# castorini/howl

Hardware: AMD Instinct MI355X
Metric: utterances/sec/node (res8 end-to-end training step, 1s@16kHz, 40-mel) (higher is better)
Workload: dtype f32; 1 GPU; res8 training step (frontend+fwd+xent+bwd+AdamW), 512 x 1 s utterances per GPU, 12 labels -- BASELINE configs[2] per-GPU share: res8 GSC-12, 512 x 1 s per GPU (4096 over 8); global_batch=512, samples_per_utterance=16000, labels=12, parallelism=single, frontend=eval

## Files before the change

howl_amd/csrc/res8.hip:

```cpp
#include "howl_common.hip.h"
#include "../../include/howl_hip.h"

namespace {

struct HowlPtrs6 {
    float* p[6];
};
constexpr int MAX_WINDOWS = 64;
struct HowlWinRows {
    int lo[MAX_WINDOWS], hi[MAX_WINDOWS];
};
struct HowlBnBuffers {
    float* running_mean;
    float* running_var;
    long long* num_batches;
};
struct BnFold {
    const float* part;
    int nparts;
    double count;
    float* stats_out;
    HowlBnBuffers bn;
};

// ... 519 lines not shown
        SlotVal v[3];
        SlotVal ge[3];
        int bsl = b, bnsl = bn, pv = P;
        bool zb = false, zn = false;
        if constexpr (HALO == 2) {
            const StripPos pb = strip_pos(gx.sg, b, P / PW), pn = strip_pos(gx.sg, more ? bn : b, P / PW);
            bsl = pb.bu, bnsl = pn.bu, pv = pb.hv * PW;
            zb = pb.hv < P / PW, zn = pn.hv < P / PW;
        }
        f32x4 acc[NTV];
        KCursor<NTV> k;
        if constexpr (NTW > 0) k_begin<NTW, TS>(k, acc, c.ltile, c.wnt, c.CS, P, c.t0, lane);
        if constexpr (NTW > 0) k_prime<NTW>(k);
        constexpr bool STAGE = true;
        const int a0 = 2, a1 = 2, a2 = KG_A - 4, b0 = 2, b1 = 2, b2 = KG_B - 4;
#define HOWL_WINO_CHUNK() ((void)0)
#define HOWL_WINO_BAR() ((void)0)
        if constexpr (STAGE) {
            slot_load<MODE, HALO>(v[0], cfg, ubase + r1, tid, pk1[0], bsl);
            slot_load<MODE, HALO>(v[1], cfg, ubase + r1, tid + CONV_THREADS, pk1[1], bsl);
            if constexpr (HALO == 1) halo_load<MODE>(v[2], cfg, (size_t)(b ^ 1) * NMAP * P, hs[1], gcol, b);
            if constexpr (HALO == 2) grid_load<MODE>(ge, cfg, gx, 1, b, P / PW, P);
        }
        HOWL_STAIR(3);
        HOWL_WINO_CHUNK();
        if constexpr (NTW > 0) k_run<NTW>(k, acc, c.CS, a0);
        HOWL_WINO_BAR();
        if constexpr (STAGE) {
            slot_write<MODE>(v[0], cfg, ubase + r1, tid, pk1[0], c.tile, c.lm, HALO == 2 && zb && ((gx.pad[1] >> 0) & 1));
            slot_write<MODE>(v[1], cfg, ubase + r1, tid + CONV_THREADS, pk1[1], c.tile, c.lm, HALO == 2 && zb && ((gx.pad[1] >> 1) & 1));
            if constexpr (HALO == 1) halo_write<MODE>(v[2], cfg, hs[1], lcol, c.tile, c.lm);
            if constexpr (HALO == 2) grid_write<MODE>(ge, cfg, gx, 1, b, P / PW, c.tile, c.lm);
            slot_load<MODE, HALO>(v[0], cfg, ubase + r1, tid + 2 * CONV_THREADS, pk1[2], bsl);
            slot_load<MODE, HALO>(v[1], cfg, ubase + r1, tid + 3 * CONV_THREADS, pk1[3], bsl);
        }
        HOWL_STAIR(2);
        HOWL_WINO_CHUNK();
        if constexpr (NTW > 0) k_run<NTW>(k, acc, c.CS, a1);
        HOWL_WINO_BAR();
        if constexpr (STAGE) {
            slot_write<MODE>(v[0], cfg, ubase + r1, tid + 2 * CONV_THREADS, pk1[2], c.tile, c.lm, HALO == 2 && zb && ((gx.pad[1] >> 2) & 1));
            slot_write<MODE>(v[1], cfg, ubase + r1, tid + 3 * CONV_THREADS, pk1[3], c.tile, c.lm, HALO == 2 && zb && ((gx.pad[1] >> 3) & 1));
        }
        HOWL_STAIR(1);
        HOWL_WINO_CHUNK();
        if constexpr (NTW > 0) k_run<NTW>(k, acc, c.CS, a2);
        HOWL_WINO_BAR();
        HOWL_STAIR(0);
        __syncthreads();
        if constexpr (NTW > 0) k_prime<NTW>(k);
        if (STAGE && more) {
            slot_load<MODE, HALO>(v[0], cfg, nbase, tid, pk0[0], bnsl);
            slot_load<MODE, HALO>(v[1], cfg, nbase, tid + CONV_THREADS, pk0[1], bnsl);
            slot_load<MODE, HALO>(v[2], cfg, nbase, tid + 2 * CONV_THREADS, pk0[2], bnsl);
            if constexpr (HALO == 2) grid_load<MODE>(ge, cfg, gx, 0, bn, P / PW, P);
        }
        HOWL_STAIR(3);
        HOWL_WINO_CHUNK();
        if constexpr (NTW > 0) k_run<NTW>(k, acc, c.CS, b0);
        HOWL_WINO_BAR();
        if (STAGE && more) {
            slot_write<MODE>(v[0], cfg, nbase, tid, pk0[0], c.tile, c.lm, HALO == 2 && zn && ((gx.pad[0] >> 0) & 1));
            slot_write<MODE>(v[1], cfg, nbase, tid + CONV_THREADS, pk0[1], c.tile, c.lm, HALO == 2 && zn && ((gx.pad[0] >> 1) & 1));
            slot_write<MODE>(v[2], cfg, nbase, tid + 2 * CONV_THREADS, pk0[2], c.tile, c.lm, HALO == 2 && zn && ((gx.pad[0] >> 2) & 1));
            if constexpr (HALO == 2) grid_write<MODE>(ge, cfg, gx, 0, bn, P / PW, c.tile, c.lm);
            slot_load<MODE, HALO>(v[0], cfg, nbase, tid + 3 * CONV_THREADS, pk0[3], bnsl);
            slot_load<MODE, HALO>(v[1], cfg, nbase, tid + 4 * CONV_THREADS, pk0[4], bnsl);
            if constexpr (HALO == 1) halo_load<MODE>(v[2], cfg, (size_t)(bn ^ 1) * NMAP * P, hs[0], gcol, bn);
        }
        HOWL_STAIR(2);
        HOWL_WINO_CHUNK();
        if constexpr (NTW > 0) k_run<NTW>(k, acc, c.CS, b1);
        HOWL_WINO_BAR();
        if (STAGE && more) {
            slot_write<MODE>(v[0], cfg, nbase, tid + 3 * CONV_THREADS, pk0[3], c.tile, c.lm, HALO == 2 && zn && ((gx.pad[0] >> 3) & 1));
            slot_write<MODE>(v[1], cfg, nbase, tid + 4 * CONV_THREADS, pk0[4], c.tile, c.lm, HALO == 2 && zn && ((gx.pad[0] >> 4) & 1));
            if constexpr (HALO == 1) halo_write<MODE>(v[2], cfg, hs[0], lcol, c.tile, c.lm);
        }
        float2 ev[NTV][2];
        if constexpr (NTW > 0) {
            if (eop != nullptr) {
                const EpiAddr<NTW, TS> ea(epi, c.t0, lane);
                const char* ebase = reinterpret_cast<const char*>(eop + ubase);
#pragma unroll
                for (int i = 0; i < NTW; ++i)
#pragma unroll
                    for (int hh = 0; hh < 2; ++hh) ev[i][hh] = *reinterpret_cast<const float2*>(ebase + ea.off(i, hh));
            }
// ... 1 lines not shown
            k_run<NTW>(k, acc, c.CS, b2);
            k_tail<NTW>(k, acc, dl);
            HOWL_STAIR(0);
        }
        if constexpr (NTW > 0) conv_epilogue<MODE, NTW, TS, HALO>(acc, ev, epi, ubase, c.t0, lane, st0, st1, b, pv);
        __syncthreads();
    }
}

struct BwdFold {
    const float* stats;
    const float* m12;
    const float* part;
    int nparts;
    double count;
};
__device__ __forceinline__ void bwd_consts_to_lds(float* lm, int ch, float mean, float rstd, float m1, float m2) {
    lm[ch] = rstd;
    lm[CP + ch] = -rstd * rstd * m2;
    lm[2 * CP + ch] = rstd * (mean * rstd * m2 - m1);
}
__device__ __forceinline__ void bwd_fold_to_lds(float* lm, const BwdFold& f, int tid, int nthreads) {
    const int lane = tid & 63, wave = tid >> 6;
    if (f.part == nullptr) {
        if (tid < CP) bwd_consts_to_lds(lm, tid, f.stats[tid], f.stats[CP + tid], f.m12[tid], f.m12[CP + tid]);
    } else {
        const int c8 = lane >> 3;
        for (int ch0 = 4 * wave; ch0 < CP; ch0 += 4 * (nthreads >> 6)) {
            const int ch = ch0 + (c8 & 3);
            const float mean = f.stats[ch], rstd = f.stats[CP + ch];
            const double acc = fold_part_column(f.part, part_stride(f.nparts), f.nparts, (c8 < 4 ? 0 : CP) + ch, lane);
            const double second = __shfl_xor(acc, 32);
            if (c8 < 4 && (lane & 7) == 0)
                bwd_consts_to_lds(lm, ch, mean, rstd, (float)(acc / f.count), (float)(second / f.count));
        }
    }
}

struct WFold {
// ... 98 lines not shown
                const float fr = (ch < NMAP) ? (float)(1.0 / sqrt(var + (double)BN_EPS)) : 0.0f;
                lm[ch] = -fm * fr;
                lm[CP + ch] = fr;
                if (bid == 0 && slice == 0) {
                    fold.stats_out[ch] = fm;
                    fold.stats_out[CP + ch] = fr;
                    if (ch < NMAP && fold.bn.running_mean != nullptr) {
                        const double unbiased = fold.count > 1.0 ? var * fold.count / (fold.count - 1.0) : var;
                        fold.bn.running_mean[ch] = (1.0f - BN_MOMENTUM) * fold.bn.running_mean[ch] + BN_MOMENTUM * (float)mean;
                        fold.bn.running_var[ch] = (1.0f - BN_MOMENTUM) * fold.bn.running_var[ch] + BN_MOMENTUM * (float)unbiased;
                    }
                    if (ch == 0 && fold.bn.num_batches != nullptr) fold.bn.num_batches[0] += 1;
                }
            }
        }
        if (MODE == 1 && cfg.fused) bwd_fold_to_lds(lm, bfold, tid, CONV_THREADS);
        zero_lds(tile, TF, tid, CONV_THREADS);
#pragma unroll
        for (int j = 0; j < 7; ++j) {
            const int i = tid + j * CONV_THREADS;
            if (i < 3 * KSTEPS * 16) reinterpret_cast<float4*>(wl)[i] = wv[j];
        }
    }
    if (MODE == 0 && !folding && tid < CP) {
        lm[tid] = cfg.affine ? -in_stats[tid] * in_stats[CP + tid] : 0.0f;
        lm[CP + tid] = cfg.affine ? in_stats[CP + tid] : 1.0f;
    }
    const int cout = 16 * nt + (lane & 15);
    const bool cvalid = cout < NMAP;
    float xshift = 0.0f, xrstd = 1.0f;
    if (MODE == 1 && xs != nullptr && xs_stats != nullptr && cvalid) {
// ... 541 lines not shown
    WSlot first[WNT];
    if (b < B) {
#pragma unroll
        for (int j = 0; j < WNT; ++j) {
            wz_load<HALO>(first[j].z, st.z, (size_t)b * NMAP * P, zt[j], ct[j], HALO == 2 ? strip_pos(sg, b, H).bu : b);
            wx_load(first[j].x, st.x, (size_t)b * NMAP * P, xt[j]);
        }
    }
    float firsth = 0.0f, firstr = 0.0f;
    if constexpr (HALO != 0) {
        if (b < B) firsth = whalo_load(st.x, (size_t)(b ^ 1) * NMAP * P, wh[0], (b & 1) ? PW - 1 : 0);
    }
    if constexpr (HALO == 2) {
        if (b < B) firstr = wrow_load(st.x, gx, b, H, P, false);
    }
    zero_lds(lds, tile_floats_z(H) + tile_floats_x(H), tid, CONV_THREADS);
    if (st.z.fused) {
        bwd_fold_to_lds(lm, bfold, tid, CONV_THREADS);
    }
    if (tid < CP) {
        lm[4 * CP + tid] = st.xaffine ? -in_stats[tid] * in_stats[CP + tid] : 0.0f;
        lm[5 * CP + tid] = st.xaffine ? in_stats[CP + tid] : 1.0f;
    }
    __syncthreads();
    if (b < B) {
#pragma unroll
        for (int j = 0; j < WNT; ++j) {
            const bool padded = HALO == 2 && strip_pos(sg, b, H).hv < H;
            wz_write(first[j].z, st.z, zt[j], ct[j], tz, lm, padded && ((gx.pzt >> j) & 1));
            wx_write(first[j].x, st.xaffine, xt[j], ct[j], tx, lm, padded && ((gx.pxt >> j) & 1));
// ... 53 lines not shown
    if (r < SD)
        conv3x3_body<1, SD, HALO>(zc, nullptr, wp, nullptr, dx, xs, xs_stats, spart, nullptr, B, H, j, nblk, r, BnFold{}, bfold, wf, sg);
    else
        wgrad_body<SW, HALO>(WStage{zc, s_prev, false}, in_stats, bfold, wpart, B, H, j, nblk, r - SD, sg);
}

struct RowsAdamW {
    float* p;
    const float* g0;
    float* m;
    float* v;
    HowlAdamWCoef c;
    long rest_lo, rest_hi;
    int on;
};
__device__ __forceinline__ void reduce_rows_body(const float* __restrict__ part, int nparts, int ncols, int mode,
                                                 float* __restrict__ out, const RowsAdamW& opt) {
    __shared__ float red[16][64];
    const int lane = threadIdx.x & 63, rg = threadIdx.x >> 6, nrg = blockDim.x >> 6;
    const int col = blockIdx.x * 64 + lane;
    float s = 0.0f;
    if (col < ncols) {
        const float* src = part + col;
        for (int g = rg; g < nparts; g += 8 * nrg) {
            float v[8];
#pragma unroll
            for (int u = 0; u < 8; ++u) {
                const int r = g + u * nrg;
                v[u] = src[(size_t)(r < nparts ? r : nparts - 1) * ncols];
            }
// ... 8 lines not shown
        for (int r = 1; r < nrg; ++r) tot += red[r][lane];
        long d = -1;
        if (mode == 0) {
            d = col;
        } else {
            const int co = col / WNCOL, idx = col - co * WNCOL;
            if (co < NMAP && idx < WTAPS) d = (co * NMAP + idx % NMAP) * 9 + idx / NMAP;
        }
        if (d >= 0) {
            out[d] = tot;
            if (opt.on) howl_adamw_element(opt.p, opt.m, opt.v, (size_t)((out - opt.g0) + d), tot, opt.c);
        }
    }
}

__global__ __launch_bounds__(1024) void reduce_rows_all_kernel(const float* __restrict__ part, size_t layer_stride, int nparts,
                                                              HowlPtrs6 out, const float* __restrict__ c0part, int c0parts,
                                                              float* __restrict__ c0out, int y0, int yskip, int nrows, RowsAdamW opt) {
    if ((int)blockIdx.y >= nrows) {
        for (long i = opt.rest_lo + (long)blockIdx.x * blockDim.x + threadIdx.x; i < opt.rest_hi; i += (long)gridDim.x * blockDim.x)
            howl_adamw_element(opt.p, opt.m, opt.v, (size_t)i, opt.g0[i], opt.c);
        return;
    }
    const int y = y0 + (int)blockIdx.y * (1 + yskip);
    if (y < 6) {
        reduce_rows_body(part + y * layer_stride, nparts, CP * WNCOL, 1, out.p[y], opt);
    } else if (blockIdx.x * 64 < NMAP * 9) {
        reduce_rows_body(c0part, c0parts, NMAP * 9, 0, c0out, opt);
    }
}

__global__ void bn_eval_stats_kernel(HowlPtrs6 rmean, HowlPtrs6 rvar, float* __restrict__ stats) {
    const int layer = blockIdx.x, c = threadIdx.x;
// ... 288 lines not shown
                    }
            }
        }
    }
#pragma unroll
    for (int j = 0; j < C0G_CPW; ++j)
#pragma unroll
        for (int t = 0; t < 9; ++t) {
            const float v = wave_sum_rows(acc[j][t]);
            if (lane == 0) part[(size_t)blockIdx.x * NMAP * 9 + (C0G_CPW * wave + j) * 9 + t] = v;
        }
}

constexpr int HEAD_XC = 64;
constexpr int HEAD_THREADS = 768, HEAD_PARTS = 16;
__global__ __launch_bounds__(HEAD_THREADS) void head_fwd_kernel(const float* __restrict__ s6, const float* __restrict__ stats,
                                                       const float* __restrict__ wout, const float* __restrict__ bout,
                                                       float* __restrict__ pooled, float* __restrict__ logits, int B,
                                                       int P, int C, const long long* __restrict__ labels,
                                                       float* __restrict__ nll, float* __restrict__ dlogits,
                                                       float* __restrict__ dpool, float inv_batch,
                                                       const float* __restrict__ pool, int npg, int npg_used, BnFold fold,
                                                       int ns ) {
    __shared__ float lp[CP];
    __shared__ float ll[HEAD_XC], dl[HEAD_XC], lse_s;
    __shared__ float lst[2 * CP];
    __shared__ float lw[HEAD_XC * NMAP];
    __shared__ float lparts[HEAD_PARTS][CP];
    const int tid = threadIdx.x, lane = tid & 63, wave = tid >> 6;
    const bool w_in_lds = C <= HEAD_XC;
    if (w_in_lds)
        for (int i = tid; i < C * NMAP; i += HEAD_THREADS) lw[i] = wout[i];
    if (fold.part != nullptr) {
        const int c8 = lane >> 3;
        for (int w0 = wave; w0 < CP / 4; w0 += HEAD_THREADS / 64) {
            const int c = 4 * w0 + (c8 & 3);
            const double sm = fold_part_column(fold.part, part_stride(fold.nparts), fold.nparts, (c8 < 4 ? 0 : CP) + c, lane);
            const double q = __shfl_xor(sm, 32);
            if (c8 < 4 && (lane & 7) == 0) {
                const double mean = sm / fold.count;
                double var = q / fold.count - mean * mean;
                var = var < 0.0 ? 0.0 : var;
                const float fm = (c < NMAP) ? (float)mean : 0.0f;
                const float fr = (c < NMAP) ? (float)(1.0 / sqrt(var + (double)BN_EPS)) : 0.0f;
                lst[c] = fm;
                lst[CP + c] = fr;
                if (blockIdx.x == 0) {
                    fold.stats_out[c] = fm;
                    fold.stats_out[CP + c] = fr;
                    if (c < NMAP && fold.bn.running_mean != nullptr) {
                        const double unbiased = fold.count > 1.0 ? var * fold.count / (fold.count - 1.0) : var;
                        fold.bn.running_mean[c] = (1.0f - BN_MOMENTUM) * fold.bn.running_mean[c] + BN_MOMENTUM * (float)mean;
                        fold.bn.running_var[c] = (1.0f - BN_MOMENTUM) * fold.bn.running_var[c] + BN_MOMENTUM * (float)unbiased;
                    }
                    if (c == 0 && fold.bn.num_batches != nullptr) fold.bn.num_batches[0] += 1;
                }
            }
        }
    } else if (tid < 2 * CP) {
        lst[tid] = stats[tid];
    }
    __syncthreads();
    for (int b = blockIdx.x; b < B; b += gridDim.x) {
        __syncthreads();
        if (pool != nullptr) {
            const int nparts = ns * npg_used;
            const int pc = tid % CP, pk = tid / CP;
            float acc = 0.0f;
            for (int k0 = 0; k0 < nparts; k0 += HEAD_PARTS) {
                const int k = k0 + pk;
                if (k < nparts) {
                    const int sgi = k / npg_used, g = k - sgi * npg_used;
                    lparts[pk][pc] = pool[(((size_t)b * ns + sgi) * npg + g) * CP + pc];
                }
                __syncthreads();
                if (tid < CP) {
// ... 57 lines not shown
        if (tid < C) {
            const float d = (expf(ll[tid] - lse_s) - (tid == y ? 1.0f : 0.0f)) * inv_batch;
            dl[tid] = d;
            dlogits[(size_t)b * C + tid] = d;
        }
        __syncthreads();
        if (tid < CP) {
            float acc = 0.0f;
            if (tid < NMAP)
                for (int k = 0; k < C; ++k) acc = fmaf(dl[k], lw[k * NMAP + tid], acc);
            dpool[(size_t)b * CP + tid] = acc;
        }
    }
}

__global__ __launch_bounds__(256) void head_fwd_windows_kernel(const float* __restrict__ s6, const float* __restrict__ stats,
                                                               const float* __restrict__ wout, const float* __restrict__ bout,
                                                               float* __restrict__ logits, int B, int nwin, int Hw,
                                                               HowlWinRows rows, float inv_count, int C, int ns) {
    __shared__ float lp[CP];
    const int tid = threadIdx.x, lane = tid & 63, wave = tid >> 6;
    const int Pw = Hw * PW;
    for (int b = blockIdx.x; b < B; b += gridDim.x) {
        __syncthreads();
        for (int c = wave; c < CP; c += 4) {
            float acc = 0.0f;
            if (c < NMAP) {
                for (int w = 0; w < nwin * ns; ++w) {
                    const float* src = s6 + ((size_t)(b * nwin * ns + w) * NMAP + c) * Pw;
                    for (int i = rows.lo[w / ns] * PW + lane; i < rows.hi[w / ns] * PW; i += 64) acc += fabsf(src[i]);
// ... 8 lines not shown
            for (int c = 0; c < NMAP; ++c) acc = fmaf(wout[k * NMAP + c], lp[c], acc);
            logits[(size_t)b * C + k] = acc;
        }
    }
}

__global__ void head_bwd_pool_kernel(const float* __restrict__ dlogits, const float* __restrict__ wout,
                                     float* __restrict__ dpool, int B, int C) {
    const int idx = blockIdx.x * blockDim.x + threadIdx.x;
    if (idx >= B * CP) return;
    const int b = idx / CP, c = idx - b * CP;
    float acc = 0.0f;
    if (c < NMAP)
        for (int k = 0; k < C; ++k) acc = fmaf(dlogits[(size_t)b * C + k], wout[k * NMAP + c], acc);
    dpool[idx] = acc;
}

__global__ __launch_bounds__(1024) void head_bwd_param_kernel(const float* __restrict__ dlogits,
                                                              const float* __restrict__ pooled,
                                                              const float* __restrict__ dpool, float* __restrict__ dwout,
                                                              float* __restrict__ dbout, float* __restrict__ m12, int B,
                                                              int C, int P, const float* __restrict__ nll,
                                                              float* __restrict__ loss) {
    __shared__ double red[2][16][64];
    if ((int)blockIdx.x == C + 1) {
        double acc = 0.0;
        for (int b = threadIdx.x; b < B; b += 1024) acc += (double)nll[b];
        acc = wave_sum_d(acc);
        if ((threadIdx.x & 63) == 0) red[0][threadIdx.x >> 6][0] = acc;
        __syncthreads();
        if (threadIdx.x == 0) {
            double tot = 0.0;
            for (int w = 0; w < 16; ++w) tot += red[0][w][0];
            loss[0] = (float)(tot / (double)B);
        }
        return;
    }
    const int k = blockIdx.x, c = threadIdx.x & 63, bg = threadIdx.x >> 6;
    double a0 = 0.0, a1 = 0.0;
    constexpr int HR = 16;
    const int cc = c < CP ? c : CP - 1;
    if (k < C) {
        for (int b = bg; b < B; b += 16 * HR) {
            float d[HR], pv[HR];
#pragma unroll
            for (int j = 0; j < HR; ++j) {
                const int bb = b + 16 * j < B ? b + 16 * j : B - 1;
                d[j] = dlogits[(size_t)bb * C + k];
                pv[j] = pooled[(size_t)bb * CP + cc];
            }
#pragma unroll
            for (int j = 0; j < HR; ++j) {
                const bool ok = b + 16 * j < B;
                a1 += ok ? (double)d[j] : 0.0;
                a0 += (ok && c < CP) ? (double)d[j] * (double)pv[j] : 0.0;
            }
        }
    } else if (c < CP) {
        for (int b = bg; b < B; b += 16 * HR) {
            float d[HR], pv[HR];
#pragma unroll
            for (int j = 0; j < HR; ++j) {
                const int bb = b + 16 * j < B ? b + 16 * j : B - 1;
                d[j] = dpool[(size_t)bb * CP + c];
                pv[j] = pooled[(size_t)bb * CP + c];
            }
#pragma unroll
            for (int j = 0; j < HR; ++j) {
                const bool ok = b + 16 * j < B;
                a0 += ok ? (double)d[j] : 0.0;
                a1 += ok ? (double)d[j] * (double)pv[j] : 0.0;
            }
        }
    }
    red[0][bg][c] = a0;
    red[1][bg][c] = a1;
    __syncthreads();
    if (bg != 0) return;
    double s0 = 0.0, s1 = 0.0;
    for (int g = 0; g < 16; ++g) {
        s0 += red[0][g][c];
        s1 += red[1][g][c];
    }
    if (k < C) {
        if (c < NMAP) dwout[k * NMAP + c] = (float)s0;
        if (c == 0) dbout[k] = (float)s1;
    } else if (c < CP) {
        const double n = (double)B * (double)P;
        m12[c] = (float)(s0 / n);
        m12[CP + c] = (float)(s1 / n);
    }
}

__global__ __launch_bounds__(1024) void xent_kernel(const float* __restrict__ logits, const long long* __restrict__ labels,
                                                    int B, int C, float* __restrict__ loss, float* __restrict__ dlogits) {
    __shared__ double red[16];
    double acc = 0.0;
    const float invB = 1.0f / (float)B;
    constexpr int XC = 32;
    for (int b = threadIdx.x; b < B; b += 1024) {
        const float* row = logits + (size_t)b * C;
        const int y = (int)labels[b];
        if (C <= XC) {
            float v[XC];
#pragma unroll
            for (int k = 0; k < XC; ++k) v[k] = row[k < C ? k : C - 1];
// ... 124 lines not shown
    return sl < 1 ? 1 : (sl > 8 ? 8 : sl);
}
bool env_off(const char* name) {
    const char* e = getenv(name);
    return e != nullptr && e[0] == '0';
}

constexpr int WIN_H = MAX_H, WIN_MARGIN = 7, WIN_STEP = WIN_H - 2 * WIN_MARGIN;
int long_windows(int H) { return H <= WIN_H ? 1 : (H - WIN_H + WIN_STEP - 1) / WIN_STEP + 1; }

struct Res8Plan {
    int B, T, M, ns, nr, Hs, hv_last, Bv, halo;
    StripGeom sg;
    int P, Pt;
    bool slicing, merged, fused;
    int G, SL;
    size_t lds_conv;
    int Bw, Tw, S0, G0, c0_nwin, c0_step, c0_last;
    bool c0_exact;
    size_t lds_conv0;
    int Gh, SD, SW, ew_grid;
    bool fold_in_pair;
    size_t wpart_stride, lds_wgrad, lds_pair;
    int S0w, G0w;
    size_t lds_conv0w;
    size_t saved_floats, train_bytes, eval_bytes;
    size_t long_map_bytes, long_bytes;
    Ws ws;
};

void plan_launches(Res8Plan& p, bool slice_conv0, char* ws_base) {
    const int cus = howl_num_cus(), H = p.Hs;
    p.P = H * PW;
    p.Pt = (p.T / 3) * PW * p.ns;
    p.saved_floats = (size_t)p.Bv * NMAP * p.P;
    p.slicing = !env_off("HOWL_RES8_SLICES");
    p.merged = !env_off("HOWL_RES8_BWD_PAIR");
    p.fused = p.halo != 0 || !env_off("HOWL_RES8_BWD_FUSED");

    p.G = even_grid(p.Bv < cus ? p.Bv : cus, p.ns);
    p.SL = p.halo == 0 && p.slicing ? conv_slices(p.G, H, cus) : 1;
    p.lds_conv = conv_lds_bytes(H, p.halo == 2);
    p.S0 = slice_conv0 && p.slicing ? conv0_slices(p.Bw, cus) : 1;
    p.G0 = p.Bw * p.S0 < 2 * cus ? p.Bw * p.S0 : 2 * cus;
    p.lds_conv0 = conv0_tile_floats(p.Tw, p.M) * sizeof(float);

    const int half = cus / 2 > 0 ? cus / 2 : 1;
    p.Gh = even_grid(p.Bv < half ? p.Bv : half, p.ns);
    p.SD = p.SW = 1;
    if (p.halo == 0 && p.slicing) pair_slices(p.Gh, H, cus, &p.SD, &p.SW);
    p.fold_in_pair = p.Gh * p.SD >= 64;
    p.wpart_stride = (size_t)p.Gh * CP * WNCOL;
    p.lds_wgrad = wgrad_lds_bytes(H);
// ... 225 lines not shown
    for (int i = 1; i <= 6; ++i) {
        Conv3x3Launch a;
        a.in = plain_tile(sv->s[i - 1]);
        a.wp = w.wp_fwd + (size_t)(i - 1) * 3 * KSTEPS * 64;
        a.res = (i % 2) == 0 ? sv->s[i - 2] : nullptr;
        a.out = sv->s[i];
        a.part = training ? ((i & 1) ? w.part : w.part2) : nullptr;
        a.pool = i == 6 ? w.pool : nullptr;
        if (i > 1 && training)
            a.fold = fold_of(i - 1, (i & 1) ? w.part2 : w.part);
        else if (i > 1)
            a.in_stats = sv->bn_stats + (size_t)(i - 2) * 2 * CP;
        HowlProfScope prof("conv3x3_fwd", stream);
        launch_conv3x3<0>(p, stream, a);
    }
    const int groups = 4 * p.SL;
    hipLaunchKernelGGL(head_fwd_kernel, dim3(B < 1024 ? B : 1024), dim3(HEAD_THREADS), 0, stream, sv->s[6],
                       sv->bn_stats + (size_t)5 * 2 * CP, prm->out_w, prm->out_b, sv->pooled, logits, B, p.Pt, C, labels, nll, dlogits,
                       w.dpool, 1.0f / (float)B, (const float*)w.pool, groups, groups < (p.P + 15) / 16 ? groups : (p.P + 15) / 16,
                       training ? fold_of(6, w.part2) : BnFold{}, p.nr * p.ns);
    HOWL_CHECK_LAUNCH("howl_res8_fwd");
    return HOWL_OK;
}

int res8_bwd_impl(const HowlRes8Params* prm, const Feat& feat, int B, int T, int M, int C, const HowlRes8Saved* sv, const float* dlogits,
                  const HowlRes8Grads* gr, void* ws, size_t ws_bytes, int part, const float* nll, float* loss, hipStream_t stream,
                  const HowlAdamW* adamw = nullptr) {
    HOWL_REQUIRE(prm && feat.x && sv && dlogits && gr && ws, "howl_res8_bwd: null pointer");
    HOWL_REQUIRE(adamw == nullptr || (part == 0 && adamw->p && adamw->g && adamw->m && adamw->v && adamw->n >= 1 && adamw->step >= 1),
                 "howl_res8_bwd: HowlAdamW needs the whole pass (part 0) and complete buffers");
    HOWL_REQUIRE(part >= 0 && part <= 2, "howl_res8_bwd_part: part must be 0 (all), 1 or 2");
    const bool run_layers = part != 2, run_conv0 = part != 1;
    HOWL_REQUIRE(mel_strips(M) > 0, "howl_res8_bwd: M must be 40 or 80 (got %d)", M);
    HOWL_REQUIRE(B >= 1 && T / 3 >= 1, "howl_res8_bwd: B=%d T=%d unsupported", B, T);
    const Res8Plan p = res8_plan(B, T, M, ws);
    HOWL_REQUIRE(p.hv_last >= 1 && p.nr <= MAX_ROW_STRIPS, "howl_res8_bwd: T=%d frames unsupported (%d row strips)", T, p.nr);
    if (int rc = check_workspace("howl_res8_bwd", ws_bytes, p.train_bytes)) return rc;
    HOWL_REQUIRE(p.saved_floats / 2 < (size_t)1 << 31, "howl_res8_bwd: B=%d too large for the 32-bit element index of the elementwise pass", B);
    const Ws& w = p.ws;
    const double count = (double)B * (double)p.Pt;

    if (run_layers) {
        if (nll == nullptr)
            hipLaunchKernelGGL(head_bwd_pool_kernel, dim3((B * CP + 255) / 256), dim3(256), 0, stream, dlogits, prm->out_w, w.dpool,
                               B, C);
        hipLaunchKernelGGL(head_bwd_param_kernel, dim3(C + (nll != nullptr ? 2 : 1)), dim3(1024), 0, stream, dlogits, sv->pooled,
                           w.dpool, gr->out_w, gr->out_b, w.m12, B, C, p.Pt, nll, loss);
    }
    float* dx_cur = nullptr;
    float* dx_next = w.bufa;
    float* ds_prev = nullptr;
    float* ds_free = w.dsa;
    for (int i = 6; i >= 1; --i) {
        const bool even = (i % 2) == 0;
        const float* stats_i = sv->bn_stats + (size_t)(i - 1) * 2 * CP;
        float* ds_out = even ? ds_free : nullptr;
        float* dz = even ? w.dz : w.dz2;
        float* part_in = p.fused ? ((i & 1) ? w.part2 : w.part) : w.part;
        float* part_out = p.fused ? ((i & 1) ? w.part : w.part2) : w.part;
        BwdLayerLaunch a;
        a.bfold = BwdFold{stats_i, w.m12, i == 6 ? (const float*)nullptr : (const float*)part_in, p.Gh * p.SD, count};
        a.zc = plain_tile(dz);
        if (p.fused)
            a.zc = StageCfg{dx_cur, sv->s[i], even ? (const float*)ds_prev : (const float*)nullptr, ds_out, w.dpool,
                            1.0f / (float)p.Pt, true, even, false};
        else if (run_layers)
            hipLaunchKernelGGL(bn_relu_bwd_kernel, dim3(p.ew_grid), dim3(BRB_THREADS), 0, stream, (const float*)dx_cur, w.dpool, sv->s[i],
                               stats_i, w.m12, a.bfold.part, p.Gh * p.SD, count, even ? (const float*)ds_prev : (const float*)nullptr,
                               even ? 1 : 0, ds_out, dz, B, p.P);
        if (even) {
            float* t = ds_prev ? ds_prev : w.dsb;
            ds_prev = ds_out;
            ds_free = t;
        }
        const bool need_stats = i > 1;
        a.s_prev = sv->s[i - 1];
// ... 14 lines not shown
                HowlProfScope prof("conv3x3_dgrad", stream);
                Conv3x3Launch d;
                d.in = a.zc, d.wp = a.wp, d.out = a.dx, d.xs = a.xs, d.xs_stats = a.xs_stats, d.part = a.spart;
                d.bfold = a.bfold, d.wf = a.wf;
                launch_conv3x3<1>(p, stream, d);
            }
            HowlProfScope prof("wgrad", stream);
            launch_wgrad(p, stream, a);
        }
        dx_cur = dx_next;
        dx_next = (dx_next == w.bufa) ? w.bufb : w.bufa;
    }
    HOWL_REQUIRE(sv->mask0 != nullptr, "howl_res8_bwd: saved->mask0 is required");
    const HowlPtrs6 gw = ptrs6(gr->conv_w);
    const RowsAdamW no_opt{nullptr, nullptr, nullptr, nullptr, HowlAdamWCoef{}, 0, 0, 0};
    const auto reduce_rows = [&](int cols, int first, int skip, int nrows, const RowsAdamW& opt) {
        hipLaunchKernelGGL(reduce_rows_all_kernel, dim3((cols + 63) / 64, nrows + (opt.on ? 1 : 0)), dim3(1024), 0, stream,
                           (const float*)w.wpart, p.wpart_stride, p.Gh, gw, (const float*)w.c0part, p.G0w, gr->conv0_w, first, skip,
                           nrows, opt);
    };
    if (part == 1)
        reduce_rows(CP * WNCOL, 0, 0, p.fold_in_pair ? 1 : 6, no_opt);
    if (run_conv0) {
        {
            HowlProfScope prof("conv0_wgrad", stream);
            launch_conv0_wgrad(p, stream, feat, sv->mask0, dx_cur);
        }
        if (part == 0) {
            RowsAdamW opt = no_opt;
            bool own_launch = adamw != nullptr;
            if (adamw != nullptr && getenv("HOWL_NO_FOLD_ADAMW") == nullptr) {
                const float* g0 = adamw->g;
                bool flat = gr->conv0_w == g0 && gr->out_b == gr->out_w + (size_t)NMAP * C &&
                            adamw->n == (size_t)NMAP * 9 + (size_t)6 * NMAP * NMAP * 9 + (size_t)NMAP * C + (size_t)C &&
                            gr->out_w == g0 + (size_t)NMAP * 9 + (size_t)6 * NMAP * NMAP * 9;
                for (int i = 0; i < 6; ++i) flat = flat && gr->conv_w[i] == g0 + (size_t)NMAP * 9 + (size_t)i * NMAP * NMAP * 9;
                if (flat) {
                    opt = RowsAdamW{adamw->p, g0, adamw->m, adamw->v,
                                    howl_adamw_coef(adamw->lr, adamw->beta1, adamw->beta2, adamw->eps, adamw->weight_decay, adamw->step,
                                                    adamw->grad_scale),
                                    (long)((p.fold_in_pair ? gr->conv_w[1] : gr->out_w) - g0), (long)adamw->n, 1};
                    own_launch = false;
                }
            }
            reduce_rows(CP * WNCOL, 0, p.fold_in_pair ? 5 : 0, p.fold_in_pair ? 2 : 7, opt);
            if (own_launch) {
                const int rc = howl_adamw_step(adamw->p, adamw->g, adamw->m, adamw->v, adamw->n, adamw->lr, adamw->beta1, adamw->beta2,
                                               adamw->eps, adamw->weight_decay, adamw->step, adamw->grad_scale, stream);
                if (rc != HOWL_OK) return rc;
            }
        } else {
            reduce_rows(NMAP * 9, 6, 0, 1, no_opt);
        }
    }
    HOWL_CHECK_LAUNCH("howl_res8_bwd");
    return HOWL_OK;
}

}

extern "C" {

size_t howl_res8_workspace_bytes(int B, int T) { return res8_plan(B, T, 40).train_bytes; }
size_t howl_res8_workspace_bytes_mels(int B, int T, int M) { return res8_plan(B, T, M).train_bytes; }
size_t howl_res8_saved_floats(int B, int T, int M) { return res8_plan(B, T, M).saved_floats; }
size_t howl_res8_eval_workspace_bytes_mels(int B, int T, int M) { return res8_plan(B, T, M).eval_bytes; }
int howl_res8_row_strips(int T) { return res8_plan(1, T, 40).nr; }
// ... 106 lines not shown
```

Baseline: 465,700 utterances/sec.

## Add wave-per-utterance head forward and optional head-grad fusion into other kernels

Adds a head forward kernel that maps one wavefront to each utterance, used by default in training when the batch is at least 512. Adds an opt-in path, selected by HOWL_RES8_HEAD_LAUNCHES=0, that removes the separate head backward parameter launch. In that path the BN mean terms are computed inside the fused conv backward prologue, and the dW/db/loss reductions and their AdamW update run as extra rows of reduce_rows_all_kernel. The aim is fewer small launches and better parallelism in the tiny head stage. The cost is redundant per-block reductions over the batch inside the conv prologue, plus more code paths to keep consistent.

```diff
diff --git a/howl_amd/csrc/res8.hip b/howl_amd/csrc/res8.hip
--- a/howl_amd/csrc/res8.hip
+++ b/howl_amd/csrc/res8.hip
@@ -557,8 +557,6 @@
         if constexpr (NTW > 0) k_prime<NTW>(k);
         constexpr bool STAGE = true;
         const int a0 = 2, a1 = 2, a2 = KG_A - 4, b0 = 2, b1 = 2, b2 = KG_B - 4;
-#define HOWL_WINO_CHUNK() ((void)0)
-#define HOWL_WINO_BAR() ((void)0)
         if constexpr (STAGE) {
             slot_load<MODE, HALO>(v[0], cfg, ubase + r1, tid, pk1[0], bsl);
             slot_load<MODE, HALO>(v[1], cfg, ubase + r1, tid + CONV_THREADS, pk1[1], bsl);
@@ -566,9 +564,7 @@
             if constexpr (HALO == 2) grid_load<MODE>(ge, cfg, gx, 1, b, P / PW, P);
         }
         HOWL_STAIR(3);
-        HOWL_WINO_CHUNK();
         if constexpr (NTW > 0) k_run<NTW>(k, acc, c.CS, a0);
-        HOWL_WINO_BAR();
         if constexpr (STAGE) {
             slot_write<MODE>(v[0], cfg, ubase + r1, tid, pk1[0], c.tile, c.lm, HALO == 2 && zb && ((gx.pad[1] >> 0) & 1));
             slot_write<MODE>(v[1], cfg, ubase + r1, tid + CONV_THREADS, pk1[1], c.tile, c.lm, HALO == 2 && zb && ((gx.pad[1] >> 1) & 1));
@@ -578,17 +574,13 @@
             slot_load<MODE, HALO>(v[1], cfg, ubase + r1, tid + 3 * CONV_THREADS, pk1[3], bsl);
         }
         HOWL_STAIR(2);
-        HOWL_WINO_CHUNK();
         if constexpr (NTW > 0) k_run<NTW>(k, acc, c.CS, a1);
-        HOWL_WINO_BAR();
         if constexpr (STAGE) {
             slot_write<MODE>(v[0], cfg, ubase + r1, tid + 2 * CONV_THREADS, pk1[2], c.tile, c.lm, HALO == 2 && zb && ((gx.pad[1] >> 2) & 1));
             slot_write<MODE>(v[1], cfg, ubase + r1, tid + 3 * CONV_THREADS, pk1[3], c.tile, c.lm, HALO == 2 && zb && ((gx.pad[1] >> 3) & 1));
         }
         HOWL_STAIR(1);
-        HOWL_WINO_CHUNK();
         if constexpr (NTW > 0) k_run<NTW>(k, acc, c.CS, a2);
-        HOWL_WINO_BAR();
         HOWL_STAIR(0);
         __syncthreads();
         if constexpr (NTW > 0) k_prime<NTW>(k);
@@ -599,9 +591,7 @@
             if constexpr (HALO == 2) grid_load<MODE>(ge, cfg, gx, 0, bn, P / PW, P);
         }
         HOWL_STAIR(3);
-        HOWL_WINO_CHUNK();
         if constexpr (NTW > 0) k_run<NTW>(k, acc, c.CS, b0);
-        HOWL_WINO_BAR();
         if (STAGE && more) {
             slot_write<MODE>(v[0], cfg, nbase, tid, pk0[0], c.tile, c.lm, HALO == 2 && zn && ((gx.pad[0] >> 0) & 1));
             slot_write<MODE>(v[1], cfg, nbase, tid + CONV_THREADS, pk0[1], c.tile, c.lm, HALO == 2 && zn && ((gx.pad[0] >> 1) & 1));
@@ -612,9 +602,7 @@
             if constexpr (HALO == 1) halo_load<MODE>(v[2], cfg, (size_t)(bn ^ 1) * NMAP * P, hs[0], gcol, bn);
         }
         HOWL_STAIR(2);
-        HOWL_WINO_CHUNK();
         if constexpr (NTW > 0) k_run<NTW>(k, acc, c.CS, b1);
-        HOWL_WINO_BAR();
         if (STAGE && more) {
             slot_write<MODE>(v[0], cfg, nbase, tid + 3 * CONV_THREADS, pk0[3], c.tile, c.lm, HALO == 2 && zn && ((gx.pad[0] >> 3) & 1));
             slot_write<MODE>(v[1], cfg, nbase, tid + 4 * CONV_THREADS, pk0[4], c.tile, c.lm, HALO == 2 && zn && ((gx.pad[0] >> 4) & 1));
@@ -646,15 +634,60 @@
     const float* part;
     int nparts;
     double count;
+    const float* hd_dpool = nullptr;
+    const float* hd_pooled = nullptr;
+    float* hd_m12 = nullptr;
+    int hd_B = 0;
 };
 __device__ __forceinline__ void bwd_consts_to_lds(float* lm, int ch, float mean, float rstd, float m1, float m2) {
     lm[ch] = rstd;
     lm[CP + ch] = -rstd * rstd * m2;
     lm[2 * CP + ch] = rstd * (mean * rstd * m2 - m1);
 }
+__device__ __forceinline__ void bwd_head_means_to_lds(float* lm, const BwdFold& f, double* scratch, int tid, bool publish) {
+    const int c = tid % CP, bg = tid / CP;
+    const int B = f.hd_B;
+    double a0 = 0.0, a1 = 0.0;
+    constexpr int HR = 16;
+    for (int b = bg; b < B; b += 16 * HR) {
+        float d[HR], pv[HR];
+#pragma unroll
+        for (int j = 0; j < HR; ++j) {
+            const int bb = b + 16 * j < B ? b + 16 * j : B - 1;
+            d[j] = f.hd_dpool[(size_t)bb * CP + c];
+            pv[j] = f.hd_pooled[(size_t)bb * CP + c];
+        }
+#pragma unroll
+        for (int j = 0; j < HR; ++j) {
+            const bool ok = b + 16 * j < B;
+            a0 += ok ? (double)d[j] : 0.0;
+            a1 += ok ? (double)d[j] * (double)pv[j] : 0.0;
+        }
+    }
+    double s[2];
+#pragma unroll
+    for (int q = 0; q < 2; ++q) {
+        scratch[bg * CP + c] = q == 0 ? a0 : a1;
+        __syncthreads();
+        double t = 0.0;
+        if (bg == 0)
+            for (int g = 0; g < 16; ++g) t += scratch[g * CP + c];
+        s[q] = t;
+        __syncthreads();
+    }
+    if (bg == 0) {
+        const float m1 = (float)(s[0] / f.count), m2 = (float)(s[1] / f.count);
+        bwd_consts_to_lds(lm, c, f.stats[c], f.stats[CP + c], m1, m2);
+        if (publish) {
+            f.hd_m12[c] = m1;
+            f.hd_m12[CP + c] = m2;
+        }
+    }
+}
 __device__ __forceinline__ void bwd_fold_to_lds(float* lm, const BwdFold& f, int tid, int nthreads) {
     const int lane = tid & 63, wave = tid >> 6;
-    if (f.part == nullptr) {
+    if (f.hd_dpool != nullptr) {
+    } else if (f.part == nullptr) {
         if (tid < CP) bwd_consts_to_lds(lm, tid, f.stats[tid], f.stats[CP + tid], f.m12[tid], f.m12[CP + tid]);
     } else {
         const int c8 = lane >> 3;
@@ -783,7 +816,11 @@
                 }
             }
         }
-        if (MODE == 1 && cfg.fused) bwd_fold_to_lds(lm, bfold, tid, CONV_THREADS);
+        if (MODE == 1 && cfg.fused) {
+            if (bfold.hd_dpool != nullptr)
+                bwd_head_means_to_lds(lm, bfold, reinterpret_cast<double*>(wl), tid, bid == 0 && slice == 0);
+            bwd_fold_to_lds(lm, bfold, tid, CONV_THREADS);
+        }
         zero_lds(tile, TF, tid, CONV_THREADS);
 #pragma unroll
         for (int j = 0; j < 7; ++j) {
@@ -1355,6 +1392,8 @@
     if constexpr (HALO == 2) {
         if (b < B) firstr = wrow_load(st.x, gx, b, H, P, false);
     }
+    if (st.z.fused && bfold.hd_dpool != nullptr)
+        bwd_head_means_to_lds(lm, bfold, reinterpret_cast<double*>(lds), tid, false);
     zero_lds(lds, tile_floats_z(H) + tile_floats_x(H), tid, CONV_THREADS);
     if (st.z.fused) {
         bwd_fold_to_lds(lm, bfold, tid, CONV_THREADS);
@@ -1438,6 +1477,110 @@
     long rest_lo, rest_hi;
     int on;
 };
+__device__ __forceinline__ void head_adamw(const RowsAdamW& opt, const float* g, float val) {
+    if (opt.on) howl_adamw_element(opt.p, opt.m, opt.v, (size_t)(g - opt.g0), val, opt.c);
+}
+struct HeadRows {
+    const float* dlogits;
+    const float* pooled;
+    const float* dpool;
+    float* dwout;
+    float* dbout;
+    int B, C, P;
+    const float* nll;
+    float* loss;
+    int on;
+};
+template <int HR>
+__device__ __forceinline__ void head_param_block(double (*red)[16][64], int blk, const float* __restrict__ dlogits,
+                                                 const float* __restrict__ pooled, const float* __restrict__ dpool,
+                                                 float* __restrict__ dwout, float* __restrict__ dbout, float* __restrict__ m12,
+                                                 int B, int C, int P, const float* __restrict__ nll, float* __restrict__ loss,
+                                                 const RowsAdamW& opt) {
+    if (blk == C + 1) {
+        double acc = 0.0;
+        for (int b = threadIdx.x; b < B; b += 1024) acc += (double)nll[b];
+        acc = wave_sum_d(acc);
+        if ((threadIdx.x & 63) == 0) red[0][threadIdx.x >> 6][0] = acc;
+        __syncthreads();
+        if (threadIdx.x == 0) {
+            double tot = 0.0;
+            for (int w = 0; w < 16; ++w) tot += red[0][w][0];
+            loss[0] = (float)(tot / (double)B);
+        }
+        return;
+    }
+    const int k = blk, c = threadIdx.x & 63, bg = threadIdx.x >> 6;
+    double a0 = 0.0, a1 = 0.0;
+    const int cc = c < CP ? c : CP - 1;
+    if (k < C) {
+        for (int b = bg; b < B; b += 16 * HR) {
+            float d[HR], pv[HR];
+#pragma unroll
+            for (int j = 0; j < HR; ++j) {
+                const int bb = b + 16 * j < B ? b + 16 * j : B - 1;
+                d[j] = dlogits[(size_t)bb * C + k];
+                pv[j] = pooled[(size_t)bb * CP + cc];
+            }
+#pragma unroll
+            for (int j = 0; j < HR; ++j) {
+                const bool ok = b + 16 * j < B;
+                a1 += ok ? (double)d[j] : 0.0;
+                a0 += (ok && c < CP) ? (double)d[j] * (double)pv[j] : 0.0;
+            }
+        }
+    } else if (c < CP) {
+        for (int b = bg; b < B; b += 16 * HR) {
+            float d[HR], pv[HR];
+#pragma unroll
+            for (int j = 0; j < HR; ++j) {
+                const int bb = b + 16 * j < B ? b + 16 * j : B - 1;
+                d[j] = dpool[(size_t)bb * CP + c];
+                pv[j] = pooled[(size_t)bb * CP + c];
+            }
+#pragma unroll
+            for (int j = 0; j < HR; ++j) {
+                const bool ok = b + 16 * j < B;
+                a0 += ok ? (double)d[j] : 0.0;
+                a1 += ok ? (double)d[j] * (double)pv[j] : 0.0;
+            }
+        }
+    }
+    red[0][bg][c] = a0;
+    red[1][bg][c] = a1;
+    __syncthreads();
+    if (bg != 0) return;
+    double s0 = 0.0, s1 = 0.0;
+    for (int g = 0; g < 16; ++g) {
+        s0 += red[0][g][c];
+        s1 += red[1][g][c];
+    }
+    if (k < C) {
+        if (c < NMAP) {
+            dwout[k * NMAP + c] = (float)s0;
+            head_adamw(opt, dwout + k * NMAP + c, (float)s0);
+        }
+        if (c == 0) {
+            dbout[k] = (float)s1;
+            head_adamw(opt, dbout + k, (float)s1);
+        }
+    } else if (c < CP) {
+        const double n = (double)B * (double)P;
+        m12[c] = (float)(s0 / n);
+        m12[CP + c] = (float)(s1 / n);
+    }
+}
+__global__ __launch_bounds__(1024) void head_bwd_param_kernel(const float* __restrict__ dlogits,
+                                                              const float* __restrict__ pooled,
+                                                              const float* __restrict__ dpool, float* __restrict__ dwout,
+                                                              float* __restrict__ dbout, float* __restrict__ m12, int B,
+                                                              int C, int P, const float* __restrict__ nll,
+                                                              float* __restrict__ loss) {
+    __shared__ double red[2][16][64];
+    head_param_block<16>(red, (int)blockIdx.x, dlogits, pooled, dpool, dwout, dbout, m12, B, C, P, nll, loss,
+                     RowsAdamW{nullptr, nullptr, nullptr, nullptr, HowlAdamWCoef{}, 0, 0, 0});
+}
+
 __device__ __forceinline__ void reduce_rows_body(const float* __restrict__ part, int nparts, int ncols, int mode,
                                                  float* __restrict__ out, const RowsAdamW& opt) {
     __shared__ float red[16][64];
@@ -1476,9 +1619,20 @@
     }
 }
 
-__global__ __launch_bounds__(1024) void reduce_rows_all_kernel(const float* __restrict__ part, size_t layer_stride, int nparts,
+__global__ __launch_bounds__(1024, 8) void reduce_rows_all_kernel(const float* __restrict__ part, size_t layer_stride, int nparts,
                                                               HowlPtrs6 out, const float* __restrict__ c0part, int c0parts,
-                                                              float* __restrict__ c0out, int y0, int yskip, int nrows, RowsAdamW opt) {
+                                                              float* __restrict__ c0out, int y0, int yskip, int nrows, RowsAdamW opt,
+                                                              HeadRows head) {
+    if (head.on && blockIdx.y + 1 == gridDim.y) {
+        __shared__ double hred[2][16][64];
+        const int nblk = head.C + (head.nll != nullptr ? 1 : 0);
+        for (int k = blockIdx.x; k < nblk; k += gridDim.x) {
+            head_param_block<8>(hred, k < head.C ? k : head.C + 1, head.dlogits, head.pooled, head.dpool, head.dwout, head.dbout,
+                             nullptr, head.B, head.C, head.P, head.nll, head.loss, opt);
+            __syncthreads();
+        }
+        return;
+    }
     if ((int)blockIdx.y >= nrows) {
         for (long i = opt.rest_lo + (long)blockIdx.x * blockDim.x + threadIdx.x; i < opt.rest_hi; i += (long)gridDim.x * blockDim.x)
             howl_adamw_element(opt.p, opt.m, opt.v, (size_t)i, opt.g0[i], opt.c);
@@ -1797,23 +1951,8 @@
 
 constexpr int HEAD_XC = 64;
 constexpr int HEAD_THREADS = 768, HEAD_PARTS = 16;
-__global__ __launch_bounds__(HEAD_THREADS) void head_fwd_kernel(const float* __restrict__ s6, const float* __restrict__ stats,
-                                                       const float* __restrict__ wout, const float* __restrict__ bout,
-                                                       float* __restrict__ pooled, float* __restrict__ logits, int B,
-                                                       int P, int C, const long long* __restrict__ labels,
-                                                       float* __restrict__ nll, float* __restrict__ dlogits,
-                                                       float* __restrict__ dpool, float inv_batch,
-                                                       const float* __restrict__ pool, int npg, int npg_used, BnFold fold,
-                                                       int ns ) {
-    __shared__ float lp[CP];
-    __shared__ float ll[HEAD_XC], dl[HEAD_XC], lse_s;
-    __shared__ float lst[2 * CP];
-    __shared__ float lw[HEAD_XC * NMAP];
-    __shared__ float lparts[HEAD_PARTS][CP];
-    const int tid = threadIdx.x, lane = tid & 63, wave = tid >> 6;
-    const bool w_in_lds = C <= HEAD_XC;
-    if (w_in_lds)
-        for (int i = tid; i < C * NMAP; i += HEAD_THREADS) lw[i] = wout[i];
+__device__ __forceinline__ void head_stats_to_lds(float* lst, const BnFold& fold, const float* __restrict__ stats, int tid) {
+    const int lane = tid & 63, wave = tid >> 6;
     if (fold.part != nullptr) {
         const int c8 = lane >> 3;
         for (int w0 = wave; w0 < CP / 4; w0 += HEAD_THREADS / 64) {
@@ -1843,6 +1982,26 @@
     } else if (tid < 2 * CP) {
         lst[tid] = stats[tid];
     }
+}
+
+__global__ __launch_bounds__(HEAD_THREADS) void head_fwd_kernel(const float* __restrict__ s6, const float* __restrict__ stats,
+                                                       const float* __restrict__ wout, const float* __restrict__ bout,
+                                                       float* __restrict__ pooled, float* __restrict__ logits, int B,
+                                                       int P, int C, const long long* __restrict__ labels,
+                                                       float* __restrict__ nll, float* __restrict__ dlogits,
+                                                       float* __restrict__ dpool, float inv_batch,
+                                                       const float* __restrict__ pool, int npg, int npg_used, BnFold fold,
+                                                       int ns ) {
+    __shared__ float lp[CP];
+    __shared__ float ll[HEAD_XC], dl[HEAD_XC], lse_s;
+    __shared__ float lst[2 * CP];
+    __shared__ float lw[HEAD_XC * NMAP];
+    __shared__ float lparts[HEAD_PARTS][CP];
+    const int tid = threadIdx.x, lane = tid & 63, wave = tid >> 6;
+    const bool w_in_lds = C <= HEAD_XC;
+    if (w_in_lds)
+        for (int i = tid; i < C * NMAP; i += HEAD_THREADS) lw[i] = wout[i];
+    head_stats_to_lds(lst, fold, stats, tid);
     __syncthreads();
     for (int b = blockIdx.x; b < B; b += gridDim.x) {
         __syncthreads();
@@ -1930,6 +2089,64 @@
     }
 }
 
+__global__ __launch_bounds__(HEAD_THREADS) void head_fwd_wave_kernel(const float* __restrict__ stats, const float* __restrict__ wout,
+                                                            const float* __restrict__ bout, float* __restrict__ pooled,
+                                                            float* __restrict__ logits, int B, int P, int C,
+                                                            const long long* __restrict__ labels, float* __restrict__ nll,
+                                                            float* __restrict__ dlogits, float* __restrict__ dpool,
+                                                            float inv_batch, const float* __restrict__ pool, int npg,
+                                                            int npg_used, BnFold fold, int ns) {
+    __shared__ float lst[2 * CP];
+    __shared__ float lw[HEAD_XC * NMAP];
+    const int tid = threadIdx.x, lane = tid & 63, wave = tid >> 6;
+    for (int i = tid; i < C * NMAP; i += HEAD_THREADS) lw[i] = wout[i];
+    head_stats_to_lds(lst, fold, stats, tid);
+    __syncthreads();
+    const int nparts = ns * npg_used;
+    const int pc = lane < CP ? lane : CP - 1;
+    const int wc = lane < NMAP ? lane : NMAP - 1;
+    const int kc = lane < C ? lane : C - 1;
+    const float mean = lst[pc], rstd = lst[CP + pc];
+    const float bias = bout[kc];
+    for (int b = blockIdx.x * (HEAD_THREADS / 64) + wave; b < B; b += gridDim.x * (HEAD_THREADS / 64)) {
+        float acc = 0.0f;
+        for (int k0 = 0; k0 < nparts; k0 += HEAD_PARTS) {
+            float pv[HEAD_PARTS];
+#pragma unroll
+            for (int j = 0; j < HEAD_PARTS; ++j) {
+                const int k = k0 + j < nparts ? k0 + j : nparts - 1;
+                const int sgi = k / npg_used, g = k - sgi * npg_used;
+                pv[j] = pool[(((size_t)b * ns + sgi) * npg + g) * CP + pc];
+            }
+#pragma unroll
+            for (int j = 0; j < HEAD_PARTS; ++j) acc = k0 + j < nparts ? acc + pv[j] : acc;
+        }
+        const float v = lane < NMAP ? (acc / (float)P - mean) * rstd : 0.0f;
+        if (lane < CP) pooled[(size_t)b * CP + lane] = v;
+        float lg = bias;
+#pragma unroll
+        for (int c = 0; c < NMAP; ++c) lg = fmaf(lw[kc * NMAP + c], __shfl(v, c), lg);
+        if (lane < C) logits[(size_t)b * C + lane] = lg;
+        if (labels == nullptr) continue;
+        const int y = (int)labels[b];
+        float mx = __shfl(lg, 0);
+        for (int k = 1; k < C; ++k) mx = fmaxf(mx, __shfl(lg, k));
+        float se = 0.0f;
+        for (int k = 0; k < C; ++k) se += expf(__shfl(lg, k) - mx);
+        const float lse = mx + logf(se);
+        const float ly = __shfl(lg, y);
+        if (lane == 0) nll[b] = lse - ly;
+        const float d = (expf(lg - lse) - (lane == y ? 1.0f : 0.0f)) * inv_batch;
+        if (lane < C) dlogits[(size_t)b * C + lane] = d;
+        float dp = 0.0f;
+        for (int k = 0; k < C; ++k) {
+            const float dk = __shfl(d, k);
+            dp = lane < NMAP ? fmaf(dk, lw[k * NMAP + wc], dp) : dp;
+        }
+        if (lane < CP) dpool[(size_t)b * CP + lane] = dp;
+    }
+}
+
 __global__ __launch_bounds__(256) void head_fwd_windows_kernel(const float* __restrict__ s6, const float* __restrict__ stats,
                                                                const float* __restrict__ wout, const float* __restrict__ bout,
                                                                float* __restrict__ logits, int B, int nwin, int Hw,
@@ -1968,82 +2185,6 @@
     if (c < NMAP)
         for (int k = 0; k < C; ++k) acc = fmaf(dlogits[(size_t)b * C + k], wout[k * NMAP + c], acc);
     dpool[idx] = acc;
-}
-
-__global__ __launch_bounds__(1024) void head_bwd_param_kernel(const float* __restrict__ dlogits,
-                                                              const float* __restrict__ pooled,
-                                                              const float* __restrict__ dpool, float* __restrict__ dwout,
-                                                              float* __restrict__ dbout, float* __restrict__ m12, int B,
-                                                              int C, int P, const float* __restrict__ nll,
-                                                              float* __restrict__ loss) {
-    __shared__ double red[2][16][64];
-    if ((int)blockIdx.x == C + 1) {
-        double acc = 0.0;
-        for (int b = threadIdx.x; b < B; b += 1024) acc += (double)nll[b];
-        acc = wave_sum_d(acc);
-        if ((threadIdx.x & 63) == 0) red[0][threadIdx.x >> 6][0] = acc;
-        __syncthreads();
-        if (threadIdx.x == 0) {
-            double tot = 0.0;
-            for (int w = 0; w < 16; ++w) tot += red[0][w][0];
-            loss[0] = (float)(tot / (double)B);
-        }
-        return;
-    }
-    const int k = blockIdx.x, c = threadIdx.x & 63, bg = threadIdx.x >> 6;
-    double a0 = 0.0, a1 = 0.0;
-    constexpr int HR = 16;
-    const int cc = c < CP ? c : CP - 1;
-    if (k < C) {
-        for (int b = bg; b < B; b += 16 * HR) {
-            float d[HR], pv[HR];
-#pragma unroll
-            for (int j = 0; j < HR; ++j) {
-                const int bb = b + 16 * j < B ? b + 16 * j : B - 1;
-                d[j] = dlogits[(size_t)bb * C + k];
-                pv[j] = pooled[(size_t)bb * CP + cc];
-            }
-#pragma unroll
-            for (int j = 0; j < HR; ++j) {
-                const bool ok = b + 16 * j < B;
-                a1 += ok ? (double)d[j] : 0.0;
-                a0 += (ok && c < CP) ? (double)d[j] * (double)pv[j] : 0.0;
-            }
-        }
-    } else if (c < CP) {
-        for (int b = bg; b < B; b += 16 * HR) {
-            float d[HR], pv[HR];
-#pragma unroll
-            for (int j = 0; j < HR; ++j) {
-                const int bb = b + 16 * j < B ? b + 16 * j : B - 1;
-                d[j] = dpool[(size_t)bb * CP + c];
-                pv[j] = pooled[(size_t)bb * CP + c];
-            }
-#pragma unroll
-            for (int j = 0; j < HR; ++j) {
-                const bool ok = b + 16 * j < B;
-                a0 += ok ? (double)d[j] : 0.0;
-                a1 += ok ? (double)d[j] * (double)pv[j] : 0.0;
-            }
-        }
-    }
-    red[0][bg][c] = a0;
-    red[1][bg][c] = a1;
-    __syncthreads();
-    if (bg != 0) return;
-    double s0 = 0.0, s1 = 0.0;
-    for (int g = 0; g < 16; ++g) {
-        s0 += red[0][g][c];
-        s1 += red[1][g][c];
-    }
-    if (k < C) {
-        if (c < NMAP) dwout[k * NMAP + c] = (float)s0;
-        if (c == 0) dbout[k] = (float)s1;
-    } else if (c < CP) {
-        const double n = (double)B * (double)P;
-        m12[c] = (float)(s0 / n);
-        m12[CP + c] = (float)(s1 / n);
-    }
 }
 
 __global__ __launch_bounds__(1024) void xent_kernel(const float* __restrict__ logits, const long long* __restrict__ labels,
@@ -2198,6 +2339,7 @@
     StripGeom sg;
     int P, Pt;
     bool slicing, merged, fused;
+    bool head_wave, head_inline;
     int G, SL;
     size_t lds_conv;
     int Bw, Tw, S0, G0, c0_nwin, c0_step, c0_last;
@@ -2221,6 +2363,9 @@
     p.slicing = !env_off("HOWL_RES8_SLICES");
     p.merged = !env_off("HOWL_RES8_BWD_PAIR");
     p.fused = p.halo != 0 || !env_off("HOWL_RES8_BWD_FUSED");
+    const char* head_launches = getenv("HOWL_RES8_HEAD_LAUNCHES");
+    p.head_wave = head_launches == nullptr ? p.B >= 512 : head_launches[0] == '0';
+    p.head_inline = head_launches != nullptr && head_launches[0] == '0' && p.fused;
 
     p.G = even_grid(p.Bv < cus ? p.Bv : cus, p.ns);
     p.SL = p.halo == 0 && p.slicing ? conv_slices(p.G, H, cus) : 1;
@@ -2476,11 +2621,19 @@
         HowlProfScope prof("conv3x3_fwd", stream);
         launch_conv3x3<0>(p, stream, a);
     }
-    const int groups = 4 * p.SL;
-    hipLaunchKernelGGL(head_fwd_kernel, dim3(B < 1024 ? B : 1024), dim3(HEAD_THREADS), 0, stream, sv->s[6],
-                       sv->bn_stats + (size_t)5 * 2 * CP, prm->out_w, prm->out_b, sv->pooled, logits, B, p.Pt, C, labels, nll, dlogits,
-                       w.dpool, 1.0f / (float)B, (const float*)w.pool, groups, groups < (p.P + 15) / 16 ? groups : (p.P + 15) / 16,
-                       training ? fold_of(6, w.part2) : BnFold{}, p.nr * p.ns);
+    const int groups = 4 * p.SL, groups_used = groups < (p.P + 15) / 16 ? groups : (p.P + 15) / 16;
+    if (training && C <= HEAD_XC && p.head_wave) {
+        const int waves = HEAD_THREADS / 64, blocks = (B + waves - 1) / waves;
+        hipLaunchKernelGGL(head_fwd_wave_kernel, dim3(blocks < 1024 ? blocks : 1024), dim3(HEAD_THREADS), 0, stream,
+                           (const float*)(sv->bn_stats + (size_t)5 * 2 * CP), prm->out_w, prm->out_b, sv->pooled, logits, B, p.Pt, C,
+                           labels, nll, dlogits, w.dpool, 1.0f / (float)B, (const float*)w.pool, groups, groups_used,
+                           fold_of(6, w.part2), p.nr * p.ns);
+    } else {
+        hipLaunchKernelGGL(head_fwd_kernel, dim3(B < 1024 ? B : 1024), dim3(HEAD_THREADS), 0, stream, sv->s[6],
+                           sv->bn_stats + (size_t)5 * 2 * CP, prm->out_w, prm->out_b, sv->pooled, logits, B, p.Pt, C, labels, nll,
+                           dlogits, w.dpool, 1.0f / (float)B, (const float*)w.pool, groups, groups_used,
+                           training ? fold_of(6, w.part2) : BnFold{}, p.nr * p.ns);
+    }
     HOWL_CHECK_LAUNCH("howl_res8_fwd");
     return HOWL_OK;
 }
@@ -2506,8 +2659,9 @@
         if (nll == nullptr)
             hipLaunchKernelGGL(head_bwd_pool_kernel, dim3((B * CP + 255) / 256), dim3(256), 0, stream, dlogits, prm->out_w, w.dpool,
                                B, C);
-        hipLaunchKernelGGL(head_bwd_param_kernel, dim3(C + (nll != nullptr ? 2 : 1)), dim3(1024), 0, stream, dlogits, sv->pooled,
-                           w.dpool, gr->out_w, gr->out_b, w.m12, B, C, p.Pt, nll, loss);
+        if (!p.head_inline)
+            hipLaunchKernelGGL(head_bwd_param_kernel, dim3(C + (nll != nullptr ? 2 : 1)), dim3(1024), 0, stream, dlogits, sv->pooled,
+                               w.dpool, gr->out_w, gr->out_b, w.m12, B, C, p.Pt, nll, loss);
     }
     float* dx_cur = nullptr;
     float* dx_next = w.bufa;
@@ -2522,6 +2676,12 @@
         float* part_out = p.fused ? ((i & 1) ? w.part : w.part2) : w.part;
         BwdLayerLaunch a;
         a.bfold = BwdFold{stats_i, w.m12, i == 6 ? (const float*)nullptr : (const float*)part_in, p.Gh * p.SD, count};
+        if (i == 6 && p.head_inline) {
+            a.bfold.hd_dpool = w.dpool;
+            a.bfold.hd_pooled = sv->pooled;
+            a.bfold.hd_m12 = w.m12;
+            a.bfold.hd_B = B;
+        }
         a.zc = plain_tile(dz);
         if (p.fused)
             a.zc = StageCfg{dx_cur, sv->s[i], even ? (const float*)ds_prev : (const float*)nullptr, ds_out, w.dpool,
@@ -2566,13 +2726,15 @@
     HOWL_REQUIRE(sv->mask0 != nullptr, "howl_res8_bwd: saved->mask0 is required");
     const HowlPtrs6 gw = ptrs6(gr->conv_w);
     const RowsAdamW no_opt{nullptr, nullptr, nullptr, nullptr, HowlAdamWCoef{}, 0, 0, 0};
-    const auto reduce_rows = [&](int cols, int first, int skip, int nrows, const RowsAdamW& opt) {
-        hipLaunchKernelGGL(reduce_rows_all_kernel, dim3((cols + 63) / 64, nrows + (opt.on ? 1 : 0)), dim3(1024), 0, stream,
+    const HeadRows head_rows{dlogits, sv->pooled, w.dpool, gr->out_w, gr->out_b, B, C, p.Pt, nll, loss, p.head_inline ? 1 : 0};
+    const HeadRows no_head{nullptr, nullptr, nullptr, nullptr, nullptr, 0, 0, 0, nullptr, nullptr, 0};
+    const auto reduce_rows = [&](int cols, int first, int skip, int nrows, const RowsAdamW& opt, const HeadRows& head) {
+        hipLaunchKernelGGL(reduce_rows_all_kernel, dim3((cols + 63) / 64, nrows + (opt.on ? 1 : 0) + head.on), dim3(1024), 0, stream,
                            (const float*)w.wpart, p.wpart_stride, p.Gh, gw, (const float*)w.c0part, p.G0w, gr->conv0_w, first, skip,
-                           nrows, opt);
+                           nrows, opt, head);
     };
     if (part == 1)
-        reduce_rows(CP * WNCOL, 0, 0, p.fold_in_pair ? 1 : 6, no_opt);
+        reduce_rows(CP * WNCOL, 0, 0, p.fold_in_pair ? 1 : 6, no_opt, head_rows);
     if (run_conv0) {
         {
             HowlProfScope prof("conv0_wgrad", stream);
@@ -2591,18 +2753,19 @@
                     opt = RowsAdamW{adamw->p, g0, adamw->m, adamw->v,
                                     howl_adamw_coef(adamw->lr, adamw->beta1, adamw->beta2, adamw->eps, adamw->weight_decay, adamw->step,
                                                     adamw->grad_scale),
-                                    (long)((p.fold_in_pair ? gr->conv_w[1] : gr->out_w) - g0), (long)adamw->n, 1};
+                                    (long)((p.fold_in_pair ? gr->conv_w[1] : gr->out_w) - g0),
+                                    p.head_inline ? (long)(gr->out_w - g0) : (long)adamw->n, 1};
                     own_launch = false;
                 }
             }
-            reduce_rows(CP * WNCOL, 0, p.fold_in_pair ? 5 : 0, p.fold_in_pair ? 2 : 7, opt);
+            reduce_rows(CP * WNCOL, 0, p.fold_in_pair ? 5 : 0, p.fold_in_pair ? 2 : 7, opt, head_rows);
             if (own_launch) {
                 const int rc = howl_adamw_step(adamw->p, adamw->g, adamw->m, adamw->v, adamw->n, adamw->lr, adamw->beta1, adamw->beta2,
                                                adamw->eps, adamw->weight_decay, adamw->step, adamw->grad_scale, stream);
                 if (rc != HOWL_OK) return rc;
             }
         } else {
-            reduce_rows(NMAP * 9, 6, 0, 1, no_opt);
+            reduce_rows(NMAP * 9, 6, 0, 1, no_opt, no_head);
         }
     }
     HOWL_CHECK_LAUNCH("howl_res8_bwd");
```

Result: no change. 467,000 utterances/sec (median of 6 runs) (+0.3%).
